# hasnainfarid/Mujoco_Gymnasium_Environments

Hardware: AMD Instinct MI355X
Metric: env steps/sec (whole node), humanoid_soccer 4096 envs/GPU at 1/2/4/8 MI355X (higher is better)
Workload: dtype f64

## Files before the change

### mujoco_gymnasium_environments_amd/csrc/mgx_api.hip

```cpp
#include <hip/hip_runtime.h>

#include <cmath>
#include <cstdio>
#include <cstring>
#include <map>
#include <mutex>
#include <string>
#include <vector>

#include "mgx_internal.h"

using namespace mgx;

MGX_PROF_SETTER(mgx_prof_set_buffer)

namespace {
thread_local std::string g_err;
int fail(int code, const std::string& msg) {
  g_err = msg;
  return code;
}
#define HIPCHK(x) MGX_HIPCHK(x)
}

// ... 543 lines not shown
  p.bcap = 32 + (p.maxE / 4) * (8 + 32 * ((nv + 7) / 8));
  p.tw = MGX_TW;
  p.nobs = nobs;
  size_t off = 0;
  auto take = [&](size_t bytes) { size_t r = off; off = (off + bytes + 255) / 256 * 256; return r; };
  size_t S = (size_t)p.S, NB = (size_t)n_env * (banks > 0 ? banks : 1);
  p.o_ctr = take(64);
  p.o_carry = take(S * p.carry_stride * rb);
  p.o_carryi = take(S * p.carryi_stride * 4);
  p.o_ne = take(S * 4); p.o_blen = take(S * 4); p.o_niter = take(S * 4); p.o_k2list = take(S * 4); p.o_k2big = take(S * 4); p.o_fix = take((size_t)n_env * 4);
  p.hmain = !rk && !cap_env && !p.sqg && !H.pgs_lds_b && p.capE < p.maxE &&
            staged_pgs_lds_bytes(m, p.maxE, pgs_lanes(), 1, mgx_twl(false)) <=
                (H.pgs_wpc == 4 ? staged_pgs_lds_bytes(m, p.capE, pgs_lanes(), 0, mgx_twl(false))
                                : 160 * 1024 / H.pgs_wpc);
  if (p.hmain) p.warena = 0;
  p.split_blocks = 0;
  const int split = H.pgs_split_blocks >= 0 ? H.pgs_split_blocks : split_default;
  if (!rk && !p.sqg && !H.pgs_lds_b && pgs_lanes() == 16 && split > 0) {
    const int one = staged_pgs_lds_bytes(m, p.maxE, 64, 0, mgx_twl(false));
    int main_lds = staged_pgs_lds_bytes(m, p.capE, 16, 0, mgx_twl(false));
    if (p.hmain) main_lds = std::max(main_lds, staged_pgs_lds_bytes(m, p.maxE, 16, 1, mgx_twl(false)));
    const bool b32 = (uint64_t)p.bcap * (uint64_t)rb < (1ull << 32);
    if (b32 && one <= (cap_env ? 160 * 1024 : main_lds)) {
      p.split_blocks = std::min(split, p.capE / 4 + 1);
      p.hmain = 0;
      p.warena = 0;
    }
  }
  p.prio_rows = H.pgs_prio_rows > 0 ? H.pgs_prio_rows : p.capE;
  p.nbk = (p.hmain || p.split_blocks ? p.maxE : p.capE) / 4 + 1;
  p.o_hist = take((size_t)(p.maxE / 4 + 1) * 4);
  p.o_blist = take((size_t)(p.maxE / 4 + 1) * S * 4);
  p.o_scal = take(S * p.maxE * MGX_SCAL * rb);
  p.o_blk = take(S * (p.maxE / 4) * p.tw * 4);
  p.o_B = take(S * (size_t)p.bcap * rb);
  p.o_vout = take(S * 64 * rb);
  p.o_bq = take(NB * nq * rb); p.o_bv = take(NB * nv * rb); p.o_ba = take(NB * nv * rb); p.o_btime = take(NB * rb);
  p.o_bobs = take(NB * nobs * 4); p.o_bprev = take(NB * 6 * rb); p.o_bwind = take(NB * 3 * rb);
  p.o_bk = take(NB * 4); p.o_bep = take(NB * 4); p.o_bwarn = take(NB * 4); p.o_bseed = take(NB * 8);
  int nb = m->precision == MGX_F32 ? m->mf.nbody : m->md.nbody;
  p.maxC = m->Ls.max_ncon;
  p.o_cpos = take(S * 3 * (size_t)p.maxC * rb);
  p.o_tq = take(nq * rb); p.o_tv = take(nv * rb); p.o_ta = take(64 * rb); p.o_tt = take(rb);
  p.o_tx = take(3 * nb * rb); p.o_txq = take(4 * nb * rb); p.o_tsc = take(3 * nb * rb); p.o_tn = take(4);
  p.o_tcg = take(2 * p.maxC * 4); p.o_tcd = take(p.maxC * rb); p.o_tcm = take(p.maxC * rb);
  p.o_rkw = take(S * 4);
  p.o_tscr = take(m->L.gB ? (size_t)m->L.gB_stride * rb : 64);
  if (rk) {
    const int nq4 = (nq + 3) & ~3;
    p.rk_stride = 2 * nq4 + 8 * 64 + 4;
    p.o_rk = take(S * p.rk_stride * rb);
    p.o_rks = take(S * 4);
  }
  if (P) *P = p;
  return off;
}
static size_t make_pipe(const mgx_model* m, void* ws, int n_env, int banks, Pipe* P) {
  return make_staged_pipe(m, ws, n_env, banks, P, false, 80, MGX_PGS_SPLIT_BLOCKS);
}

int mgx::staged_pgs_lds_bytes(const mgx_model* m, int rows, int lps, int sqg, int twl) {
  int rb = m->precision == MGX_F32 ? 4 : 8;
  int nb3 = (rows / 4 + MGX_PGS_RING - 1) / MGX_PGS_RING * MGX_PGS_RING;
  const int spw = 64 / lps;
  const int sq = sqg ? 4 : 4 * MGX_SCAL;
  return spw * (sq * nb3 + 4) * rb + spw * nb3 * 4 * twl + 64;
}
static int pgs_lds_bytes(const mgx_model* m, int rows, int sqg = 0) {
  return staged_pgs_lds_bytes(m, rows, pgs_lanes(), sqg, mgx_twl(false));
}

mgx::Hooks mgx::read_hooks() {
  Hooks h;
  auto get = [](const char* name, int dflt) {
    const char* v = getenv(name);
    return v && *v ? atoi(v) : dflt;
  };
  h.pgs_lds_rows = get("MGX_PGS_LDS_ROWS", 0);
  h.rk_lds_rows = get("MGX_RK_LDS_ROWS", 0);
  h.pgs_single = get("MGX_PGS_SINGLE", 0);
  h.pgs_lds_b = get("MGX_PGS_LDS_B", MGX_PGS_LDS_B) != 0;
  h.pgs_arena = get("MGX_PGS_ARENA", 0);
  h.pgs_lds_pad = get("MGX_PGS_LDS_PAD", 0);
  h.pgs_wide_lds = get("MGX_PGS_WIDE_LDS", 1);
  h.pgs_spw = get("MGX_PGS_SPW", 0);
  h.pgs_prio_rows = get("MGX_PGS_PRIO_ROWS", 0);
  h.pgs_split_blocks = get("MGX_PGS_SPLIT_BLOCKS", -1);
  h.tight_bp = get("MGX_TIGHT_BROADPHASE", -1);
  h.pgs_wpc = get("MGX_PGS_WPC", 4);
  if (h.pgs_wpc < 4 || h.pgs_wpc > 16) h.pgs_wpc = 4;
  h.side_stream = get("MGX_SIDE_STREAM", 1) != 0;
  h.gcon = get("MGX_GCON", 1);
  h.rows_lds = get("MGX_ROWS_LDS", 0);
  return h;
}

struct SideStream {
  hipStream_t s;
  hipEvent_t rows, big;
};
static SideStream* side_stream(hipStream_t st) {
  static std::mutex mu;
  static std::map<std::pair<hipStream_t, int>, SideStream*> cache;
  int dev = 0;
  if (hipGetDevice(&dev) != hipSuccess) return nullptr;
  std::lock_guard<std::mutex> lock(mu);
  auto key = std::make_pair(st, dev);
  auto it = cache.find(key);
  if (it != cache.end()) return it->second;
  SideStream* x = new SideStream{};
  if (hipStreamCreateWithFlags(&x->s, hipStreamNonBlocking) != hipSuccess ||
      hipEventCreateWithFlags(&x->rows, hipEventDisableTiming) != hipSuccess ||
      hipEventCreateWithFlags(&x->big, hipEventDisableTiming) != hipSuccess) {
    delete x;
    x = nullptr;
  }
  cache[key] = x;
  return x;
}

static int settle_lds_bytes(const mgx_model* m, const Pipe& P) {
  int b = pgs_lds_bytes(m, P.maxE);
  if (m->Ls.bytes > b) b = m->Ls.bytes;
  if (m->Lf.bytes > b) b = m->Lf.bytes;
  return b;
}

template <typename T>
static int soccer_step_staged(const mgx_model* m, const DevModel<T>& M, const DevModel<T>& Ms, const DevModel<T>& Mf,
                              const SoccerIds<T>& ids, const mgx_state* s, const mgx_soccer_env* e, const float* action,
                              float* obs, double* reward, uint8_t* terminated, uint8_t* truncated, float* final_obs,
                              int autoreset, uint64_t seed, int env_offset, int n_env, const uint8_t* mask,
                              hipStream_t st) {
  Pipe P;
  int banks = autoreset ? e->banks : 0;
  size_t need = make_pipe(m, e->workspace, n_env, e->banks, &P);
  if (e->workspace_bytes < need) return fail(MGX_E_ARG, "workspace smaller than mgx_soccer_workspace_bytes");
  int slots = n_env * (1 + banks);
  const Hooks& H = m->hooks;
  const int rlds = H.rows_lds > m->Ls.bytes && H.rows_lds <= 64 * 1024 ? H.rows_lds : m->Ls.bytes;
  launch_soccer_rows<T>(Ms, ids, *s, *e, action, n_env, mask, P, banks, slots, rlds, st);
  T scale = (T)1 / (M.meaninertia * (T)(M.nv > 1 ? M.nv : 1));
  const int wgrid = 64 / pgs_lanes() * MGX_PGS_WIDE_GRID, wlds = pgs_lds_bytes(m, P.maxE);
  int mlds = H.pgs_lds_b ? P.arena : pgs_lds_bytes(m, P.capE, P.sqg);
  if (P.hmain) mlds = std::max(mlds, pgs_lds_bytes(m, P.maxE, 1));
  if (P.split_blocks) mlds = std::max(mlds, staged_pgs_lds_bytes(m, P.maxE, 64, 0, mgx_twl(false)));
  if (H.pgs_lds_pad > mlds && H.pgs_lds_pad <= 96 * 1024) mlds = H.pgs_lds_pad;
  if (!H.pgs_lds_b && (P.maxE <= P.capE || P.hmain || P.split_blocks)) {
    launch_pgs<T>(P, slots, mlds, st, M.iterations, M.tolerance, scale, 0, H);
  } else if (SideStream* side = (!H.pgs_lds_b && H.side_stream) ? side_stream(st) : nullptr) {
    HIPCHK(hipEventRecord(side->rows, st));
    HIPCHK(hipStreamWaitEvent(side->s, side->rows, 0));
    launch_pgs<T>(P, wgrid, wlds, side->s, M.iterations, M.tolerance, scale, 1, H);
    HIPCHK(hipEventRecord(side->big, side->s));
    launch_pgs<T>(P, slots, mlds, st, M.iterations, M.tolerance, scale, 0, H);
    HIPCHK(hipStreamWaitEvent(st, side->big, 0));
  } else {
    launch_pgs<T>(P, slots, mlds, st, M.iterations, M.tolerance, scale, 0, H);
    launch_pgs<T>(P, wgrid, wlds, st, M.iterations, M.tolerance, scale, 1, H);
  }
  launch_soccer_finish<T>(Mf, ids, *s, *e, action, obs, reward, terminated, truncated, final_obs, autoreset, seed,
                          env_offset, n_env, mask, P, banks, m->Lf.bytes, st);
  int fgrid = n_env < 256 ? n_env : 256;
  launch_soccer_settle<T>(Ms, Mf, ids, *s, *e, (const T*)nullptr, obs, seed, env_offset, n_env, nullptr, P, SETTLE_FIXUP,
                          fgrid, settle_lds_bytes(m, P), st, M.iterations, M.tolerance, scale);
  HIPCHK(hipGetLastError());
  return MGX_OK;
}

template <typename T>
static int soccer_reset_staged(const mgx_model* m, const DevModel<T>& M, const DevModel<T>& Ms, const DevModel<T>& Mf,
                               const SoccerIds<T>& ids, const mgx_state* s, const mgx_soccer_env* e, const T* draws,
                               float* obs, uint64_t seed, int env_offset, int n_env, const uint8_t* mask, hipStream_t st) {
  Pipe P;
  size_t need = make_pipe(m, e->workspace, n_env, e->banks, &P);
  if (e->workspace_bytes < need) return fail(MGX_E_ARG, "workspace smaller than mgx_soccer_workspace_bytes");
  T scale = (T)1 / (M.meaninertia * (T)(M.nv > 1 ? M.nv : 1));
  launch_soccer_settle<T>(Ms, Mf, ids, *s, *e, draws, obs, seed, env_offset, n_env, mask, P, SETTLE_RESET, n_env,
                          settle_lds_bytes(m, P), st, M.iterations, M.tolerance, scale);
  HIPCHK(hipGetLastError());
  return MGX_OK;
}

template <typename T>
static void fill_ids(SoccerIds<T>& o, const mgx_soccer_ids* ids, const DevModel<T>& M, const mgx_model_desc* unused) {
  (void)unused;
  o.torso = ids->torso; o.ball = ids->ball; o.goalkeeper = ids->goalkeeper; o.ball_geom = ids->ball_geom;
  o.right_foot = ids->right_foot; o.left_foot = ids->left_foot; o.field_geom = ids->field_geom;
  o.ball_qposadr = ids->ball_qposadr; o.ball_dofadr = ids->ball_dofadr; o.gk_qposadr = ids->gk_qposadr;
  o.gk_qfrc_index = ids->gk_dofadr; o.max_episode_steps = ids->max_episode_steps;
  for (int i = 0; i < 25; i++) {
    o.obs_qposadr[i] = ids->obs_jnt_qposadr[i];
    o.obs_dofadr[i] = ids->obs_jnt_dofadr[i];
    o.obs_lo[i] = (T)ids->obs_jnt_range[2 * i];
    o.obs_hi[i] = (T)ids->obs_jnt_range[2 * i + 1];
// ... 180 lines not shown
    hipLaunchKernelGGL((k_soccer<float, 0>), dim3(n_env), dim3(64), m->L.bytes, st, m->mf, m->sf, *s, *e, action,
                       (const float*)nullptr, obs, reward, terminated, truncated, final_obs, autoreset, seed,
                       env_offset, n_env, mask, none, 0);
  else
    hipLaunchKernelGGL((k_soccer<double, 0>), dim3(n_env), dim3(64), m->L.bytes, st, m->md, m->sd, *s, *e, action,
                       (const double*)nullptr, obs, reward, terminated, truncated, final_obs, autoreset, seed,
                       env_offset, n_env, mask, none, 0);
  HIPCHK(hipGetLastError());
  return MGX_OK;
}

int mgx_soccer_reset(const mgx_model* m, const mgx_state* s, const mgx_soccer_env* e, const void* draws, float* obs,
                     uint64_t seed, int env_offset, int n_env, const uint8_t* mask, void* stream) {
  if (!m || !e || !obs) return fail(MGX_E_ARG, "null argument");
  if (!m->soccer_ok) return fail(MGX_E_ARG, "mgx_soccer_configure not called");
  if (!draws && !e->episode) return fail(MGX_E_ARG, "device draws need the episode counter buffer");
  int rc = check_state(s);
  if (rc) return rc;
  if (n_env <= 0) return MGX_OK;
  hipStream_t st = (hipStream_t)stream;
  if (e->workspace) {
    if (!m->staged_ok) return fail(MGX_E_UNSUPPORTED, "staged step: model exceeds the staged solver's capacity");
    if (e->banks < 0 || e->banks > 16) return fail(MGX_E_ARG, "banks must be in [0, 16]");
    if (m->precision == MGX_F32)
      return soccer_reset_staged<float>(m, m->mf, m->mfs, m->mff, m->sf, s, e, (const float*)draws, obs, seed,
                                        env_offset, n_env, mask, st);
    return soccer_reset_staged<double>(m, m->md, m->mds, m->mdf, m->sd, s, e, (const double*)draws, obs, seed,
                                       env_offset, n_env, mask, st);
  }
  Pipe none{};
  if (m->precision == MGX_F32)
    hipLaunchKernelGGL((k_soccer<float, 1>), dim3(n_env), dim3(64), m->L.bytes, st, m->mf, m->sf, *s, *e,
                       (const float*)nullptr, (const float*)draws, obs, (double*)nullptr, (uint8_t*)nullptr,
                       (uint8_t*)nullptr, (float*)nullptr, 0, seed, env_offset, n_env, mask, none, 0);
  else
    hipLaunchKernelGGL((k_soccer<double, 1>), dim3(n_env), dim3(64), m->L.bytes, st, m->md, m->sd, *s, *e,
                       (const float*)nullptr, (const double*)draws, obs, (double*)nullptr, (uint8_t*)nullptr,
                       (uint8_t*)nullptr, (float*)nullptr, 0, seed, env_offset, n_env, mask, none, 0);
  HIPCHK(hipGetLastError());
  return MGX_OK;
}

int64_t mgx_soccer_workspace_bytes(const mgx_model* m, int n_env, int banks) {
  if (!m || n_env <= 0 || banks < 0 || banks > 16) return fail(MGX_E_ARG, "bad argument");
  if (!m->staged_ok) return fail(MGX_E_UNSUPPORTED, "staged step: model exceeds the staged solver's capacity");
  return (int64_t)make_pipe(m, nullptr, n_env, banks, nullptr);
}

int mgx_soccer_workspace_layout(const mgx_model* m, int n_env, int banks, int64_t* out, int n_out) {
  if (!m || !out || n_env <= 0 || banks < 0 || banks > 16 || n_out < 10) return fail(MGX_E_ARG, "bad argument");
  if (!m->staged_ok) return fail(MGX_E_UNSUPPORTED, "staged step: model exceeds the staged solver's capacity");
  Pipe P;
  make_pipe(m, nullptr, n_env, banks, &P);
  const int64_t v[11] = {(int64_t)P.o_ctr, (int64_t)P.o_ne, (int64_t)P.o_k2list, (int64_t)P.o_blk, (int64_t)P.o_B,
                         P.bcap, P.maxE, P.capE, P.S, m->precision == MGX_F32 ? 4 : 8, (int64_t)P.o_k2big};
  for (int i = 0; i < (n_out < 11 ? n_out : 11); i++) out[i] = v[i];
  return MGX_OK;
}

int mgx_soccer_workspace_init(const mgx_model* m, void* workspace, uint64_t bytes, int n_env, int banks, void* stream) {
  if (!m || !workspace || n_env <= 0 || banks < 0 || banks > 16) return fail(MGX_E_ARG, "bad argument");
  Pipe P;
  size_t need = make_pipe(m, workspace, n_env, banks, &P);
  if (bytes < need) return fail(MGX_E_ARG, "workspace smaller than mgx_soccer_workspace_bytes");
  hipStream_t st = (hipStream_t)stream;
  HIPCHK(hipMemsetAsync(workspace, 0, need, st));
  size_t nb = (size_t)n_env * (banks > 0 ? banks : 1);
  HIPCHK(hipMemsetAsync(P.base + P.o_bk, 0xFF, nb * 4, st));
  if (m->precision == MGX_F32)
    hipLaunchKernelGGL(k_soccer_template<float>, dim3(1), dim3(64), m->L.bytes, st, m->mf, P);
  else
    hipLaunchKernelGGL(k_soccer_template<double>, dim3(1), dim3(64), m->L.bytes, st, m->md, P);
  HIPCHK(hipGetLastError());
  return MGX_OK;
}

int mgx_soccer_logic_test(const mgx_model* m, const mgx_soccer_logic_io* io, int n_env, void* stream) {
  if (!m || !io) return fail(MGX_E_ARG, "null argument");
  if (!m->soccer_ok) return fail(MGX_E_ARG, "mgx_soccer_configure not called");
  if (io->max_contacts > m->L.max_ncon) return fail(MGX_E_CAPACITY, "max_contacts exceeds the contact capacity");
  if (n_env <= 0) return MGX_OK;
  hipStream_t st = (hipStream_t)stream;
  if (m->precision == MGX_F32)
    hipLaunchKernelGGL(k_soccer_logic<float>, dim3(n_env), dim3(64), m->L.bytes, st, m->mf, m->sf, *io, n_env);
  else
    hipLaunchKernelGGL(k_soccer_logic<double>, dim3(n_env), dim3(64), m->L.bytes, st, m->md, m->sd, *io, n_env);
  HIPCHK(hipGetLastError());
  return MGX_OK;
}

}
```

### mujoco_gymnasium_environments_amd/csrc/mgx_internal.h

```cpp
#pragma once
#include <hip/hip_runtime.h>

#include <string>

#include "../../include/mgx.h"
#include "mgx_bipedal.h"
#include "mgx_construction.h"
#include "mgx_dancing.h"
#include "mgx_martial.h"
#include "mgx_parkour.h"
#include "mgx_staged.h"

namespace mgx {
struct Hooks {
  int pgs_lds_rows = 0;
  int rk_lds_rows = 0;
  int pgs_single = 0;
  int pgs_lds_b = 0;
  int pgs_arena = 0;
  int pgs_lds_pad = 0;
  int pgs_wide_lds = 1;
  int pgs_spw = 0;
  int pgs_wpc = 4;
  int pgs_prio_rows = 0;
  int pgs_split_blocks = -1;
  int tight_bp = -1;
  int side_stream = 1;
  int gcon = 1;
  int rows_lds = 0;
};
Hooks read_hooks();
struct RayState;
struct SensorState;
}

struct mgx_model {
  mgx::Hooks hooks;
  int precision;
  int device;
  void* dbuf = nullptr;
  size_t dbytes = 0;
  mgx::DevModel<float> mf, mfs, mff;
  mgx::DevModel<double> md, mds, mdf;
  mgx::Layout L, Ls, Lf;
  bool soccer_ok = false;
  mgx::SoccerIds<float> sf;
  mgx::SoccerIds<double> sd;
  bool parkour_ok = false;
  mgx::ParkourIds<float> pkf;
  mgx::ParkourIds<double> pkd;
  bool martial_ok = false;
  mgx::MartialIds ma;
  bool bipedal_ok = false;
  mgx::BipedalIds bp;
  bool dancing_ok = false;
  mgx::DancingIds dn;
  bool assembly_ok = false;
  mgx_assembly_ids as;
  bool construction_ok = false;
  mgx::ConstructionIds cn;
  int npair;
  bool wide = false;
  bool staged_ok = false;
  bool staged_rk_ok = false;
  mgx::RayState* ray = nullptr;
  mgx::SensorState* sensor = nullptr;
};

namespace mgx {
struct DbgOff {
  int xpos, xquat, xipos, subtree_com, cinert, cdof, qM, qLD, geom_xpos, geom_xmat, ncon, con_dist, con_pos,
      con_frame, con_geom, nefc, efc_type, efc_id, efc_pos, efc_margin, efc_R, efc_aref, Bmat, cvel, cdof_dot,
      qfrc_smooth, qacc_smooth, efc_force, qacc, qfrc_constraint, niter, total;
};
inline DbgOff dbg_offsets(int nb, int nv, int nM, int ng, int C, int E) {
  DbgOff o;
  int p = 0;
  auto take = [&](int n) { int r = p; p += n; return r; };
  o.xpos = take(3 * nb); o.xquat = take(4 * nb); o.xipos = take(3 * nb); o.subtree_com = take(3 * nb);
  o.cinert = take(10 * nb); o.cdof = take(6 * nv); o.qM = take(nM); o.qLD = take(nM);
  o.geom_xpos = take(3 * ng); o.geom_xmat = take(9 * ng); o.ncon = take(1); o.con_dist = take(C);
  o.con_pos = take(3 * C); o.con_frame = take(9 * C); o.con_geom = take(2 * C); o.nefc = take(1);
  o.efc_type = take(E); o.efc_id = take(E); o.efc_pos = take(E); o.efc_margin = take(E); o.efc_R = take(E);
  o.efc_aref = take(E); o.Bmat = take(E * nv); o.cvel = take(6 * nb); o.cdof_dot = take(6 * nv);
  o.qfrc_smooth = take(nv); o.qacc_smooth = take(nv); o.efc_force = take(E); o.qacc = take(nv);
  o.qfrc_constraint = take(nv); o.niter = take(1); o.total = p;
  return o;
}
int wide_step(const mgx_model* m, const mgx_state* s, const mgx_frames& fr, int n_env, int nsub, const uint8_t* mask,
              hipStream_t st);
int wide_debug(const mgx_model* m, const mgx_state* s, int n_env, void* dbg, const DbgOff& o, hipStream_t st);
int wide_kernels_configure(const mgx_model* m);
int host_fail(int code, const std::string& msg);
int host_check_state(const mgx_state* s);
int step_kernels_configure(const mgx_model* m);
template <typename T>
void launch_pgs(const Pipe& P, int slots, int lds, hipStream_t st, int maxit, T tol, T scale, int big, const Hooks& h);
int pgs_configure_lds(int precision, int bytes, int wide);
template <typename T>
void launch_soccer_rows(const DevModel<T>& Ms, const SoccerIds<T>& ids, const mgx_state& s, const mgx_soccer_env& ev,
                        const float* action, int n_env, const uint8_t* mask, const Pipe& P, int banks, int slots, int lds,
                        hipStream_t st);
template <typename T>
void launch_soccer_finish(const DevModel<T>& Mf, const SoccerIds<T>& ids, const mgx_state& s, const mgx_soccer_env& ev,
                          const float* action, float* obs, double* reward, uint8_t* terminated, uint8_t* truncated,
                          float* final_obs, int autoreset, uint64_t seed, int env_offset, int n_env, const uint8_t* mask,
                          const Pipe& P, int banks, int lds, hipStream_t st);
template <typename T>
void launch_soccer_settle(const DevModel<T>& Ms, const DevModel<T>& Mf, const SoccerIds<T>& ids, const mgx_state& s,
                          const mgx_soccer_env& ev, const T* draws, float* obs, uint64_t seed, int env_offset, int n_env,
                          const uint8_t* mask, const Pipe& P, int mode, int grid, int lds, hipStream_t st, int maxit, T tol,
                          T scale);
int staged_kernels_configure(int precision, int ls, int lf, int settle);
size_t make_staged_pipe(const mgx_model* m, void* ws, int n_env, int banks, Pipe* P, bool rk, int nobs,
                        int split_default = 0);
int staged_pgs_lds_bytes(const mgx_model* m, int rows, int lps, int sqg, int twl);
int bipedal_staged_configure(const mgx_model* m);
int bipedal_step_staged(const mgx_model* m, const mgx_state* s, const mgx_bipedal_env* e, const float* action, float* obs,
                        double* reward, uint8_t* terminated, uint8_t* truncated, float* final_obs, int autoreset,
                        uint64_t seed, int env_offset, int n_env, const uint8_t* mask, hipStream_t st);
int bipedal_reset_staged(const mgx_model* m, const mgx_state* s, const mgx_bipedal_env* e, const void* draws,
                         float* obs, uint64_t seed, int env_offset, int n_env, const uint8_t* mask, hipStream_t st);
int64_t bipedal_workspace_bytes(const mgx_model* m, int n_env, int banks);
int bipedal_workspace_init(const mgx_model* m, void* workspace, uint64_t bytes, int n_env, int banks, hipStream_t st);
bool parkour_staged_ok(const mgx_model* m);
int parkour_staged_configure(const mgx_model* m);
int parkour_step_staged(const mgx_model* m, const mgx_state* s, const mgx_parkour_env* e, const float* action, float* obs,
                        double* reward, uint8_t* terminated, uint8_t* truncated, float* final_obs, int autoreset,
                        uint64_t seed, int env_offset, int n_env, const uint8_t* mask, hipStream_t st);
int parkour_reset_staged(const mgx_model* m, const mgx_state* s, const mgx_parkour_env* e, const void* draws,
                         float* obs, uint64_t seed, int env_offset, int n_env, const uint8_t* mask, hipStream_t st);
int64_t parkour_workspace_bytes(const mgx_model* m, int n_env, int banks);
int parkour_workspace_init(const mgx_model* m, void* workspace, uint64_t bytes, int n_env, int banks, hipStream_t st);
int pgs_lanes();
void ray_release(mgx_model* m);
void sensor_release(mgx_model* m);
int forward_kernels_configure(const mgx_model* m);
int dyn_kernels_configure(const mgx_model* m);
}

#define MGX_WIDE_MSG "nv > 64: this model runs on the wide (two dofs per lane) kernels only"

#define MGX_HIPCHK(x)                                                                                   \
  do {                                                                                                  \
    hipError_t _e = (x);                                                                                \
    if (_e != hipSuccess) return mgx::host_fail(MGX_E_HIP, std::string(#x) + ": " + hipGetErrorString(_e)); \
  } while (0)

template <typename KernelT>
int mgx_set_lds(KernelT k, int bytes) {
  if (bytes > 64 * 1024) MGX_HIPCHK(hipFuncSetAttribute((const void*)k, hipFuncAttributeMaxDynamicSharedMemorySize, bytes));
  return MGX_OK;
}
```

### mujoco_gymnasium_environments_amd/csrc/mgx_pgs.hip

```cpp
#include "mgx_internal.h"

namespace mgx {

int pgs_lanes() {
  static const int lanes = [] {
    const char* v = getenv("MGX_PGS_LPS");
    const int x = v ? atoi(v) : MGX_PGS_LPS;
    return x == 64 ? 64 : 16;
  }();
  return lanes;
}
template <typename T, int LPS, bool BLDS, bool SQG = false>
static void launch_lps(const Pipe& P, int slots, int lds, hipStream_t st, int maxit, T tol, T scale, int big,
                       int spw_hook, int spw_force = 0) {
  const int spw = spw_force ? spw_force : spw_hook ? spw_hook : 64 / LPS;
  int grid = (slots + (spw < 0 ? -spw : spw) - 1) / (spw < 0 ? -spw : spw);
  switch ((P.dpl + LPS / 8 - 1) / (LPS / 8)) {
#define MGX_PGS_CASE(E)                                                                                          \
    case E:                                                                                                     \
      hipLaunchKernelGGL((k_pgs_groups<T, E, LPS, BLDS, SQG>), dim3(grid), dim3(64), lds, st, P, maxit, tol, scale, spw, \
                         big);                                                                                  \
      break;
    MGX_PGS_CASE(1)
    default:
      if constexpr (LPS == 16) {
        switch ((P.dpl + 1) / 2) { MGX_PGS_CASE(2) MGX_PGS_CASE(3) MGX_PGS_CASE(4) default: break; }
      }
      break;
#undef MGX_PGS_CASE
  }
}

template <typename T>
void launch_pgs(const Pipe& P, int slots, int lds, hipStream_t st, int maxit, T tol, T scale, int big, const Hooks& h) {
  if (big && P.warena > 0 && pgs_lanes() == 16) {
    launch_lps<T, 16, true>(P, MGX_PGS_WIDE_LDS_GRID, P.warena + 64, st, maxit, tol, scale, big, h.pgs_spw, 1);
    return;
  }
  const bool blds = !big && h.pgs_lds_b;
  const int sp = h.pgs_spw;
  if (pgs_lanes() == 64) {
    if (blds) launch_lps<T, 64, true>(P, slots, lds, st, maxit, tol, scale, big, sp);
    else launch_lps<T, 64, false>(P, slots, lds, st, maxit, tol, scale, big, sp);
  } else {
    if (blds) launch_lps<T, 16, true>(P, slots, lds, st, maxit, tol, scale, big, sp);
    else if (P.sqg && !big) launch_lps<T, 16, false, true>(P, slots, lds, st, maxit, tol, scale, big, sp);
    else launch_lps<T, 16, false>(P, slots, lds, st, maxit, tol, scale, big, sp);
  }
}
template void launch_pgs<float>(const Pipe&, int, int, hipStream_t, int, float, float, int, const Hooks&);
template void launch_pgs<double>(const Pipe&, int, int, hipStream_t, int, double, double, int, const Hooks&);

template <typename T>
__global__ void __launch_bounds__(64) k_soccer_rows(DevModel<T> m, SoccerIds<T> ids, mgx_state s, mgx_soccer_env ev,
                                                    const float* action, int n_env, const uint8_t* mask, Pipe P,
                                                    int banks) {
  extern __shared__ __attribute__((aligned(16))) char smem[];
  int b = blockIdx.x;
  int slot;
  Env<T> e;
  if (b < n_env) {
    if (mask && !mask[b]) return;
    env_bind(m, e, smem);
    bind_carry_tail(m, e, P, b);
    load_state(m, e, (T*)s.qpos, (T*)s.qvel, (T*)s.qacc_warmstart, (T*)s.ctrl, (T*)s.qfrc_applied, (T*)s.xfrc_applied,
               (T*)s.time, b);
    soccer_pre(m, e, ids, SoccerAct(action, ev.action_f64, b, m.nu), (T*)ev.prev_ball_pos + 3 * (size_t)b,
               (T*)ev.wind + 3 * (size_t)b);
    slot = b;
  } else {
    int bi = b - n_env;
    if (!banks || bi >= n_env * P.R) return;
    int k = P.at<int>(P.o_bk)[bi];
    if (k < 0 || k >= 10) return;
    env_bind(m, e, smem);
    bind_carry_tail(m, e, P, b);
    bank_load_state(m, e, P, bi);
    slot = b;
  }
  int warn = 0;
  if (any_bad(e.qpos, m.nq)) { reset_env(m, e); warn++; }
  if (any_bad(e.qvel, m.nv)) { reset_env(m, e); warn++; }
  stage_rows(m, e, P, slot, warn);
}

template <typename T>
__global__ void __launch_bounds__(64) k_soccer_bank_finish(DevModel<T> m, SoccerIds<T> ids, int n_env, Pipe P) {
  extern __shared__ __attribute__((aligned(16))) char smem[];
  const int bi = blockIdx.x;
  if (bi >= n_env * P.R) return;
  int k = P.at<int>(P.o_bk)[bi];
  if (k < 0 || k >= 10) return;
  Env<T> e;
  env_bind(m, e, smem);
  const int slot = n_env + bi;
  int warn = load_carry(m, e, P, slot);
  if (!finish_physics(m, e, P, slot)) {
    load_template(m, e, P);
    warn++;
  }
  bank_store_state(m, e, P, bi, warn);
  k++;
  if (k == 10) bank_finalize(m, e, ids, P, bi);
  if (lane_id() == 0) P.at<int>(P.o_bk)[bi] = k;
}

template <typename T>
__global__ void __launch_bounds__(64) k_soccer_finish(DevModel<T> m, SoccerIds<T> ids, mgx_state s, mgx_soccer_env ev,
                                                      const float* action, float* obs, double* reward,
                                                      uint8_t* terminated, uint8_t* truncated, float* final_obs,
                                                      int autoreset, uint64_t seed, int env_offset, int n_env,
                                                      const uint8_t* mask, Pipe P, int banks) {
  extern __shared__ __attribute__((aligned(16))) char smem[];
  int env = blockIdx.x;
  if (env >= n_env) return;
  int l = lane_id();
  if (env == 0 && l == 0) {
    P.ctr()[3] = P.ctr()[1];
    P.ctr()[4] = P.ctr()[2];
    P.ctr()[1] = 0;
    P.ctr()[2] = 0;
  }
  if (env == 0)
    for (int b = lane_id(); b < P.nbk; b += 64) P.at<int>(P.o_hist)[b] = 0;
  Env<T> e;
  env_bind(m, e, smem);
  if (mask && !mask[env]) return;
  int warn = load_carry(m, e, P, env);
  if (!finish_physics(m, e, P, env)) {
    load_template(m, e, P);
    warn++;
  }
  store_state(m, e, (T*)s.qpos, (T*)s.qvel, (T*)s.qacc_warmstart, (T*)s.ctrl, (T*)s.qfrc_applied, (T*)s.xfrc_applied,
              (T*)s.time, env);
  if (l == 0 && s.warning) s.warning[env] += warn;
  if (l == 0 && s.overflow && e.overflow) s.overflow[env] += 1;
  const SoccerAct a(action, ev.action_f64, env, m.nu);
  float* o = obs + (size_t)env * 80;
  bool done = soccer_post(m, e, ids, a, ev.step + env, ev.goal_scored + env, (T*)ev.prev_ball_pos + 3 * (size_t)env,
                          (T*)ev.prev_robot_pos + 3 * (size_t)env, (T*)ev.stats + 5 * (size_t)env, o, reward + env,
                          terminated + env, truncated + env, ev.flags ? ev.flags + 2 * (size_t)env : nullptr);
  if (ev.rollout && l == 0) {
    double* ro = (double*)ev.rollout + 8 * (size_t)env;
    const double ne = e.nefc, it = e.nefc > 0 ? P.at<int>(P.o_niter)[env] : 0;
    ro[0] += reward[env];
    ro[1] += terminated[env];
    ro[2] += truncated[env];
    ro[3] += 1.0;
    ro[4] += ne;
    ro[5] += it;
    ro[6] += ne * ne;
    ro[7] += it * ne * ne;
  }
  if (done && autoreset) {
    if (final_obs)
      for (int i = l; i < 80; i += 64) final_obs[(size_t)env * 80 + i] = o[i];
    __threadfence();
    wsync();
    bool ok = banks && bank_install(m, e, ids, P, s, ev, obs, seed, env_offset, env);
    if (!ok && l == 0) {
      int i = atomicAdd(P.ctr(), 1);
      P.at<int>(P.o_fix)[i] = env * 4 + FIX_RESET;
    }
  }
}


template <typename T>
void launch_soccer_rows(const DevModel<T>& Ms, const SoccerIds<T>& ids, const mgx_state& s, const mgx_soccer_env& ev,
                        const float* action, int n_env, const uint8_t* mask, const Pipe& P, int banks, int slots, int lds,
                        hipStream_t st) {
  hipLaunchKernelGGL(k_soccer_rows<T>, dim3(slots), dim3(64), lds, st, Ms, ids, s, ev, action, n_env, mask, P, banks);
}
template <typename T>
void launch_soccer_finish(const DevModel<T>& Mf, const SoccerIds<T>& ids, const mgx_state& s, const mgx_soccer_env& ev,
                          const float* action, float* obs, double* reward, uint8_t* terminated, uint8_t* truncated,
                          float* final_obs, int autoreset, uint64_t seed, int env_offset, int n_env, const uint8_t* mask,
                          const Pipe& P, int banks, int lds, hipStream_t st) {
  if (banks && P.R > 0)
    hipLaunchKernelGGL(k_soccer_bank_finish<T>, dim3(n_env * P.R), dim3(64), lds, st, Mf, ids, n_env, P);
  hipLaunchKernelGGL(k_soccer_finish<T>, dim3(n_env), dim3(64), lds, st, Mf, ids, s, ev, action, obs, reward, terminated,
                     truncated, final_obs, autoreset, seed, env_offset, n_env, mask, P, banks);
}
template <typename T>
void launch_soccer_settle(const DevModel<T>& Ms, const DevModel<T>& Mf, const SoccerIds<T>& ids, const mgx_state& s,
                          const mgx_soccer_env& ev, const T* draws, float* obs, uint64_t seed, int env_offset, int n_env,
                          const uint8_t* mask, const Pipe& P, int mode, int grid, int lds, hipStream_t st, int maxit, T tol,
                          T scale) {
#define MGX_SETTLE(E, L)                                                                                            \
  hipLaunchKernelGGL((k_soccer_settle<T, E, L>), dim3(grid), dim3(64), lds, st, Ms, Mf, ids, s, ev, draws, obs, seed, \
                     env_offset, n_env, mask, P, mode, maxit, tol, scale)
  if (pgs_lanes() == 64) {
    MGX_SETTLE(1, 64);
  } else {
    switch ((P.dpl + 1) / 2) {
      case 1: MGX_SETTLE(1, 16); break;
      case 2: MGX_SETTLE(2, 16); break;
      case 3: MGX_SETTLE(3, 16); break;
      default: MGX_SETTLE(4, 16); break;
    }
  }
#undef MGX_SETTLE
}
#define MGX_STAGED_INST(T)                                                                                              \
  template void launch_soccer_rows<T>(const DevModel<T>&, const SoccerIds<T>&, const mgx_state&, const mgx_soccer_env&, \
                                      const float*, int, const uint8_t*, const Pipe&, int, int, int, hipStream_t);      \
  template void launch_soccer_finish<T>(const DevModel<T>&, const SoccerIds<T>&, const mgx_state&,                      \
                                        const mgx_soccer_env&, const float*, float*, double*, uint8_t*, uint8_t*, float*, \
                                        int, uint64_t, int, int, const uint8_t*, const Pipe&, int, int, hipStream_t);     \
  template void launch_soccer_settle<T>(const DevModel<T>&, const DevModel<T>&, const SoccerIds<T>&, const mgx_state&, \
                                        const mgx_soccer_env&, const T*, float*, uint64_t, int, int, const uint8_t*,    \
                                        const Pipe&, int, int, int, hipStream_t, int, T, T);
MGX_STAGED_INST(float)
MGX_STAGED_INST(double)
#undef MGX_STAGED_INST

int staged_kernels_configure(int precision, int ls, int lf, int settle) {
  int rc = 0;
#define MGX_SETTLE_SET(T) \
  rc |= mgx_set_lds(k_soccer_settle<T, 1, 16>, settle) | mgx_set_lds(k_soccer_settle<T, 2, 16>, settle) | \
        mgx_set_lds(k_soccer_settle<T, 3, 16>, settle) | mgx_set_lds(k_soccer_settle<T, 4, 16>, settle) | \
        mgx_set_lds(k_soccer_settle<T, 1, 64>, settle);
  if (precision == MGX_F32) {
    rc |= mgx_set_lds(k_soccer_rows<float>, ls > 64 * 1024 ? ls : 64 * 1024) | mgx_set_lds(k_soccer_finish<float>, lf) |
          mgx_set_lds(k_soccer_bank_finish<float>, lf);
    MGX_SETTLE_SET(float)
  } else {
    rc |= mgx_set_lds(k_soccer_rows<double>, ls > 64 * 1024 ? ls : 64 * 1024) | mgx_set_lds(k_soccer_finish<double>, lf) |
          mgx_set_lds(k_soccer_bank_finish<double>, lf);
    MGX_SETTLE_SET(double)
  }
#undef MGX_SETTLE_SET
  return rc;
}

int pgs_configure_lds(int precision, int pl, int wl) {
  int rc = 0;
#define MGX_PGS_SET(T, E, L)                                                                            \
  rc |= mgx_set_lds(k_pgs_groups<T, E, L, true>, pl > wl ? pl : wl) | mgx_set_lds(k_pgs_groups<T, E, L, false>, pl) | \
        mgx_set_lds(k_pgs_groups<T, E, L, false, true>, pl);
#define MGX_PGS_SET_ALL(T) \
  MGX_PGS_SET(T, 1, 16) MGX_PGS_SET(T, 2, 16) MGX_PGS_SET(T, 3, 16) MGX_PGS_SET(T, 4, 16) MGX_PGS_SET(T, 1, 64)
  if (precision == MGX_F32) { MGX_PGS_SET_ALL(float) } else { MGX_PGS_SET_ALL(double) }
#undef MGX_PGS_SET_ALL
#undef MGX_PGS_SET
  return rc;
}

}

MGX_PROF_SETTER(mgx_prof_set_buffer_pgs)
```

### mujoco_gymnasium_environments_amd/csrc/mgx_staged.h

```cpp
#pragma once
#include "mgx_soccer.h"

namespace mgx {

#define MGX_SCAL 5
#define MGX_SQ(k, i) (4 * (k) + (i))
#define MGX_TW 4
__host__ __device__ constexpr int mgx_twl(bool dofb) { return dofb ? 4 : 8; }
#define MGX_PGS_LPS 16
#define MGX_PGS_LDS_B 0
#define MGX_PGS_RING 2
#define MGX_PGS_RING_LDS 2
#define MGX_PGS_LDS_ROWS 192
#define MGX_PGS_SPLIT_BLOCKS 40
#define MGX_PGS_WIDE_GRID 256
#define MGX_PGS_WIDE_LDS_GRID 32
#define MGX_PGS_ARENA_F64 49152
#define MGX_PGS_ARENA_F32 32768
enum { FIX_RESET = 2 };

struct Pipe {
  char* base;
  int N, R, S, maxE, dpl, nv;
  int carry_stride;
  int carryi_stride;
  int bcap;
  int capE;
  int arena;
  int sqg;
  int prio_rows;
  int hmain;
  int split_blocks;
  int warena;
  size_t o_cpos;
  size_t o_carry, o_carryi, o_ne, o_blen, o_niter, o_k2list, o_k2big, o_ctr, o_fix, o_scal, o_blk, o_B, o_vout;
  int nbk;
  size_t o_hist, o_blist;
  size_t o_bq, o_bv, o_ba, o_btime, o_bobs, o_bprev, o_bwind, o_bk, o_bep, o_bwarn, o_bseed;
  size_t o_tq, o_tv, o_ta, o_tt, o_tx, o_txq, o_tsc, o_tn, o_tcg, o_tcd, o_tcm;
  int maxC;
  int tw;
  int nobs;
  int rk_stride;
  size_t o_rk, o_rks, o_rkw, o_tscr;
  template <typename X> __device__ __forceinline__ X* at(size_t off) const { return reinterpret_cast<X*>(base + off); }
  __device__ __forceinline__ int* ctr() const { return at<int>(o_ctr); }
};

template <typename T>
__device__ __forceinline__ void bind_carry_tail(const DevModel<T>& m, Env<T>& e, const Pipe& P, int slot) {
  if (m.L.carry_lds < m.L.carry_reals) {
    T* cr = P.at<T>(P.o_carry) + (size_t)slot * P.carry_stride;
    e.xfrc = cr + (m.L.xfrc - m.L.qpos);
    e.qMH = cr + (m.L.qMH - m.L.qpos);
    e.con_mu = cr + (m.L.con_mu - m.L.qpos);
  }
  if (m.L.gcon) e.con_pos = P.at<T>(P.o_cpos) + (size_t)slot * 3 * P.maxC;
}

template <typename T>
__device__ __forceinline__ int rows_plan(const DevModel<T>& m, Env<T>& e, int* nlim_out, int* ncon_out) {
  int l = lane_id();
  const int maxE = m.L.max_nefc;
  int nlim = 0;
  for (int base = 0; base < m.njnt; base += 64) {
    int j = base + l;
    bool lo = false, hi = false;
    if (j < m.njnt && m.jnt_limited[j] && (m.jnt_type[j] == JHINGE || m.jnt_type[j] == JSLIDE)) {
      T val = e.qpos[m.jnt_qposadr[j]], margin = m.jnt_margin[j];
      lo = val - m.jnt_range[2 * j] < margin;
      hi = m.jnt_range[2 * j + 1] - val < margin;
    }
    int total;
    int off = wave_excl_scan((int)lo + (int)hi, &total);
    int r = nlim + off;
    if (lo) { if (r < maxE) e.efc_id[r] = 2 * j; r++; }
    if (hi) { if (r < maxE) e.efc_id[r] = 2 * j + 1; }
    nlim += total;
  }
  if (nlim > maxE) { nlim = maxE; e.overflow |= 4; }
  int nlim4 = (nlim + 3) & ~3;
  int ncf = e.ncon;
  if (nlim4 + 4 * ncf > maxE) { ncf = (maxE - nlim4) / 4; e.overflow |= 4; }
  *nlim_out = nlim;
  *ncon_out = ncf;
  wsync();
  return nlim4 + 4 * ncf;
}

template <typename T>
__device__ __forceinline__ void rows_impedance(const DevModel<T>& m, Env<T>& e, int ne, int nlim, int nlim4, T* scal) {
  const int l = lane_id();
  for (int r = l; r < ne; r += 64) {
    const T *solref = nullptr, *solimp = nullptr;
    T pos = 0, margin = 0, diag = 0;
    if (r < nlim) {
      int code = e.efc_id[r];
// ... 892 lines not shown
    e.con_geom[2 * k + 1] = P.at<int>(P.o_tcg)[2 * k + 1];
    e.con_dist[k] = P.at<T>(P.o_tcd)[k];
    e.con_mu[k] = P.at<T>(P.o_tcm)[k];
  }
  e.qacc_ws = l < m.nv ? P.at<T>(P.o_ta)[l] : (T)0;
  e.qfrc_applied = 0;
  e.time = P.at<T>(P.o_tt)[0];
  wsync();
}

template <typename T>
__device__ __forceinline__ bool finish_physics(const DevModel<T>& m, Env<T>& e, const Pipe& P, int slot) {
  int l = lane_id();
  const bool dl = l < m.nv;
  if (e.nefc > 0) {
    T v = dl ? P.at<T>(P.o_vout)[(size_t)slot * 64 + l] : (T)0;
    T D = dl ? e.qLD[m.dof_Madr[l]] : (T)1;
    T sqrtD = sqrt(D);
    T z = dl ? v / sqrtD : (T)0;
    z = solve_L(m, e, e.qLD, z);
    e.qacc = e.qacc_smooth + z;
    e.qfrc_constraint = mul_LT(m, e, e.qLD, dl ? sqrtD * v : (T)0);
  } else {
    e.qacc = e.qacc_smooth;
    e.qfrc_constraint = 0;
  }
  if (ballot(dl && isbad(e.qacc)) != 0ull) return false;
  e.qacc_ws = e.qacc;
  euler(m, e);
  return true;
}

template <typename T>
__device__ __forceinline__ void copy_g(T* dst, const T* src, int n) {
  for (int k = lane_id(); k < n; k += 64) dst[k] = src[k];
}

template <typename T>
__device__ __forceinline__ void bank_init_draws(const DevModel<T>& m, Env<T>& e, const SoccerIds<T>& ids, const Pipe& P,
                                                int bi, int episode, uint64_t seed) {
  int l = lane_id();
  soccer_apply_reset(m, e, ids, e.vec1, P.at<T>(P.o_bwind) + 3 * (size_t)bi);
  copy_g(P.at<T>(P.o_bq) + (size_t)bi * m.nq, e.qpos, m.nq);
  if (l < m.nv) {
    P.at<T>(P.o_bv)[(size_t)bi * m.nv + l] = 0;
    P.at<T>(P.o_ba)[(size_t)bi * m.nv + l] = 0;
  }
  if (l == 0) {
    P.at<T>(P.o_btime)[bi] = 0;
    P.at<int>(P.o_bwarn)[bi] = 0;
    P.at<int>(P.o_bep)[bi] = episode;
    P.at<uint64_t>(P.o_bseed)[bi] = seed;
    P.at<int>(P.o_bk)[bi] = 0;
  }
  wsync();
}
template <typename T>
__device__ __forceinline__ void bank_init(const DevModel<T>& m, Env<T>& e, const SoccerIds<T>& ids, const Pipe& P, int env,
                                          int b, int episode, uint64_t seed, int env_offset) {
  soccer_philox_draws(seed, (uint32_t)(env_offset + env), (uint32_t)episode, ids.n_noise, e.vec1);
  wsync();
  bank_init_draws(m, e, ids, P, env * P.R + b, episode, seed);
}

template <typename T>
__device__ __forceinline__ void bank_finalize(const DevModel<T>& m, Env<T>& e, const SoccerIds<T>& ids, const Pipe& P, int bi) {
  soccer_obs(m, e, ids, 0, P.at<float>(P.o_bobs) + (size_t)bi * 80);
  int l = lane_id();
  T* pv = P.at<T>(P.o_bprev) + (size_t)bi * 6;
  if (l < 3) { pv[l] = e.xpos[3 * ids.ball + l]; pv[3 + l] = e.xpos[3 * ids.torso + l]; }
}

template <typename T>
__device__ __forceinline__ void bank_store_state(const DevModel<T>& m, Env<T>& e, const Pipe& P, int bi, int warn) {
  wsync();
  int l = lane_id();
  copy_g(P.at<T>(P.o_bq) + (size_t)bi * m.nq, e.qpos, m.nq);
  if (l < m.nv) {
    P.at<T>(P.o_bv)[(size_t)bi * m.nv + l] = e.qvel[l];
    P.at<T>(P.o_ba)[(size_t)bi * m.nv + l] = e.qacc_ws;
  }
  if (l == 0) {
    P.at<T>(P.o_btime)[bi] = e.time;
    P.at<int>(P.o_bwarn)[bi] += warn;
  }
}

template <typename T>
__device__ __forceinline__ void bank_load_state(const DevModel<T>& m, Env<T>& e, const Pipe& P, int bi) {
  int l = lane_id();
  const T* q = P.at<T>(P.o_bq) + (size_t)bi * m.nq;
  for (int k = l; k < m.nq; k += 64) e.qpos[k] = q[k];
  for (int k = l; k < m.nv; k += 64) e.qvel[k] = P.at<T>(P.o_bv)[(size_t)bi * m.nv + k];
  for (int k = l; k < m.nu; k += 64) e.ctrl[k] = 0;
  for (int k = l; k < 6 * m.nbody; k += 64) e.xfrc[k] = 0;
  e.qacc_ws = l < m.nv ? P.at<T>(P.o_ba)[(size_t)bi * m.nv + l] : (T)0;
  e.qfrc_applied = 0;
  e.time = P.at<T>(P.o_btime)[bi];
  wsync();
}

template <typename T>
__device__ __forceinline__ void bank_copy_live(const DevModel<T>& m, const Pipe& P, mgx_state s, mgx_soccer_env ev,
                                               float* obs, int env, int bi, int E) {
  int l = lane_id();
  copy_g((T*)s.qpos + (size_t)env * m.nq, P.at<T>(P.o_bq) + (size_t)bi * m.nq, m.nq);
// ... 128 lines not shown
```

Measured before the change: 1.715 million.

## Run autoreset bank pipeline on a separate low-priority stream

Splits the staged soccer step so that live-env rows and PGS run on the main stream while the reset-bank rows, PGS and bank-finish run concurrently on a low-priority side stream, using separate counters and lists in the workspace. A per-bank staging flag records which banks ran so bank-finish does not need to recheck the step counter. This is meant to hide the bank work behind the live-env solve instead of serialising it into one large grid. It adds extra workspace, events and cross-stream synchronisation, and the change in launch shapes and priorities could reduce occupancy or cause contention.

After: 1.770 million, median of 6. 3.2% higher.

```diff
diff --git a/mujoco_gymnasium_environments_amd/csrc/mgx_api.hip b/mujoco_gymnasium_environments_amd/csrc/mgx_api.hip
--- a/mujoco_gymnasium_environments_amd/csrc/mgx_api.hip
+++ b/mujoco_gymnasium_environments_amd/csrc/mgx_api.hip
@@ -619,6 +619,11 @@
     p.o_rk = take(S * p.rk_stride * rb);
     p.o_rks = take(S * 4);
   }
+  p.o_ctr2 = take(64);
+  p.o_hist2 = take((size_t)(p.maxE / 4 + 1) * 4);
+  p.o_blist2 = take((size_t)(p.maxE / 4 + 1) * NB * 4);
+  p.o_k2list2 = take(NB * 4); p.o_k2big2 = take(NB * 4);
+  p.o_bstg = take(NB * 4);
   if (P) *P = p;
   return off;
 }
@@ -657,6 +662,8 @@
   h.pgs_wpc = get("MGX_PGS_WPC", 4);
   if (h.pgs_wpc < 4 || h.pgs_wpc > 16) h.pgs_wpc = 4;
   h.side_stream = get("MGX_SIDE_STREAM", 1) != 0;
+  h.bank_stream = get("MGX_BANK_STREAM", -1);
+  if (h.bank_stream < -1 || h.bank_stream > 2) h.bank_stream = 0;
   h.gcon = get("MGX_GCON", 1);
   h.rows_lds = get("MGX_ROWS_LDS", 0);
   return h;
@@ -686,6 +693,42 @@
   return x;
 }
 
+struct BankStream {
+  hipStream_t s;
+  hipEvent_t entry, rows, live, done;
+};
+static BankStream* bank_stream(hipStream_t st) {
+  static std::mutex mu;
+  static std::map<std::pair<hipStream_t, int>, BankStream*> cache;
+  int dev = 0;
+  if (hipGetDevice(&dev) != hipSuccess) return nullptr;
+  std::lock_guard<std::mutex> lock(mu);
+  auto key = std::make_pair(st, dev);
+  auto it = cache.find(key);
+  if (it != cache.end()) return it->second;
+  BankStream* x = new BankStream{};
+  int least = 0, greatest = 0;
+  if (hipDeviceGetStreamPriorityRange(&least, &greatest) != hipSuccess ||
+      hipStreamCreateWithPriority(&x->s, hipStreamNonBlocking, least) != hipSuccess ||
+      hipEventCreateWithFlags(&x->entry, hipEventDisableTiming) != hipSuccess ||
+      hipEventCreateWithFlags(&x->rows, hipEventDisableTiming) != hipSuccess ||
+      hipEventCreateWithFlags(&x->live, hipEventDisableTiming) != hipSuccess ||
+      hipEventCreateWithFlags(&x->done, hipEventDisableTiming) != hipSuccess) {
+    (void)hipGetLastError();
+    delete x;
+    x = nullptr;
+  }
+  cache[key] = x;
+  return x;
+}
+static Pipe bank_view(const Pipe& P) {
+  Pipe B = P;
+  B.o_ctr = P.o_ctr2; B.o_hist = P.o_hist2; B.o_blist = P.o_blist2; B.o_k2list = P.o_k2list2; B.o_k2big = P.o_k2big2;
+  B.S = P.N * (P.R > 0 ? P.R : 1);
+  B.prio_rows = P.maxE;
+  return B;
+}
+
 static int settle_lds_bytes(const mgx_model* m, const Pipe& P) {
   int b = pgs_lds_bytes(m, P.maxE);
   if (m->Ls.bytes > b) b = m->Ls.bytes;
@@ -706,8 +749,47 @@
   int slots = n_env * (1 + banks);
   const Hooks& H = m->hooks;
   const int rlds = H.rows_lds > m->Ls.bytes && H.rows_lds <= 64 * 1024 ? H.rows_lds : m->Ls.bytes;
+  T scale = (T)1 / (M.meaninertia * (T)(M.nv > 1 ? M.nv : 1));
+  int bmode = banks > 0 && H.side_stream && !H.pgs_lds_b && !H.pgs_single &&
+                      (P.maxE <= P.capE || P.hmain || P.split_blocks)
+                  ? (H.bank_stream >= 0 ? H.bank_stream : m->precision == MGX_F32 ? 0 : MGX_BANK_STREAM) : 0;
+  BankStream* bs = bmode ? bank_stream(st) : nullptr;
+  if (bs) {
+    const Pipe B = bank_view(P);
+    const int nbank = n_env * P.R;
+    if (!H.pgs_prio_rows && P.split_blocks) P.prio_rows = 4 * P.split_blocks - 1;
+    int mlds = pgs_lds_bytes(m, P.capE, P.sqg);
+    if (P.hmain) mlds = std::max(mlds, pgs_lds_bytes(m, P.maxE, 1));
+    if (P.split_blocks) mlds = std::max(mlds, staged_pgs_lds_bytes(m, P.maxE, 64, 0, mgx_twl(false)));
+    if (H.pgs_lds_pad > mlds && H.pgs_lds_pad <= 96 * 1024) mlds = H.pgs_lds_pad;
+    HIPCHK(hipEventRecord(bs->entry, st));
+    launch_soccer_rows<T>(Ms, ids, *s, *e, action, n_env, mask, P, 0, n_env, rlds, st);
+    HIPCHK(hipStreamWaitEvent(bs->s, bs->entry, 0));
+    launch_soccer_rows<T>(Ms, ids, *s, *e, action, n_env, nullptr, B, banks, nbank, rlds, bs->s, n_env);
+    if (bmode == 2) HIPCHK(hipEventRecord(bs->rows, bs->s));
+    launch_pgs<T>(B, nbank, mlds, bs->s, M.iterations, M.tolerance, scale, 0, H);
+    if (bmode == 1) {
+      launch_soccer_bank_finish<T>(Mf, ids, n_env, B, 1, m->Lf.bytes, bs->s);
+      HIPCHK(hipEventRecord(bs->done, bs->s));
+    }
+    launch_pgs<T>(P, n_env, mlds, st, M.iterations, M.tolerance, scale, 0, H);
+    HIPCHK(hipStreamWaitEvent(st, bmode == 1 ? bs->done : bs->rows, 0));
+    launch_soccer_finish<T>(Mf, ids, *s, *e, action, obs, reward, terminated, truncated, final_obs, autoreset, seed,
+                            env_offset, n_env, mask, P, banks, m->Lf.bytes, st, false);
+    int fgrid = n_env < 256 ? n_env : 256;
+    launch_soccer_settle<T>(Ms, Mf, ids, *s, *e, (const T*)nullptr, obs, seed, env_offset, n_env, nullptr, P,
+                            SETTLE_FIXUP, fgrid, settle_lds_bytes(m, P), st, M.iterations, M.tolerance, scale);
+    if (bmode == 2) {
+      HIPCHK(hipEventRecord(bs->live, st));
+      HIPCHK(hipStreamWaitEvent(bs->s, bs->live, 0));
+      launch_soccer_bank_finish<T>(Mf, ids, n_env, B, 1, m->Lf.bytes, bs->s);
+      HIPCHK(hipEventRecord(bs->done, bs->s));
+      HIPCHK(hipStreamWaitEvent(st, bs->done, 0));
+    }
+    HIPCHK(hipGetLastError());
+    return MGX_OK;
+  }
   launch_soccer_rows<T>(Ms, ids, *s, *e, action, n_env, mask, P, banks, slots, rlds, st);
-  T scale = (T)1 / (M.meaninertia * (T)(M.nv > 1 ? M.nv : 1));
   const int wgrid = 64 / pgs_lanes() * MGX_PGS_WIDE_GRID, wlds = pgs_lds_bytes(m, P.maxE);
   int mlds = H.pgs_lds_b ? P.arena : pgs_lds_bytes(m, P.capE, P.sqg);
   if (P.hmain) mlds = std::max(mlds, pgs_lds_bytes(m, P.maxE, 1));
@@ -994,9 +1076,10 @@
   if (!m->staged_ok) return fail(MGX_E_UNSUPPORTED, "staged step: model exceeds the staged solver's capacity");
   Pipe P;
   make_pipe(m, nullptr, n_env, banks, &P);
-  const int64_t v[11] = {(int64_t)P.o_ctr, (int64_t)P.o_ne, (int64_t)P.o_k2list, (int64_t)P.o_blk, (int64_t)P.o_B,
-                         P.bcap, P.maxE, P.capE, P.S, m->precision == MGX_F32 ? 4 : 8, (int64_t)P.o_k2big};
-  for (int i = 0; i < (n_out < 11 ? n_out : 11); i++) out[i] = v[i];
+  const int64_t v[13] = {(int64_t)P.o_ctr, (int64_t)P.o_ne, (int64_t)P.o_k2list, (int64_t)P.o_blk, (int64_t)P.o_B,
+                         P.bcap, P.maxE, P.capE, P.S, m->precision == MGX_F32 ? 4 : 8, (int64_t)P.o_k2big,
+                         (int64_t)P.o_ctr2, (int64_t)P.o_k2list2};
+  for (int i = 0; i < (n_out < 13 ? n_out : 13); i++) out[i] = v[i];
   return MGX_OK;
 }
 
diff --git a/mujoco_gymnasium_environments_amd/csrc/mgx_internal.h b/mujoco_gymnasium_environments_amd/csrc/mgx_internal.h
--- a/mujoco_gymnasium_environments_amd/csrc/mgx_internal.h
+++ b/mujoco_gymnasium_environments_amd/csrc/mgx_internal.h
@@ -26,6 +26,7 @@
   int pgs_split_blocks = -1;
   int tight_bp = -1;
   int side_stream = 1;
+  int bank_stream = 0;
   int gcon = 1;
   int rows_lds = 0;
 };
@@ -100,12 +101,15 @@
 template <typename T>
 void launch_soccer_rows(const DevModel<T>& Ms, const SoccerIds<T>& ids, const mgx_state& s, const mgx_soccer_env& ev,
                         const float* action, int n_env, const uint8_t* mask, const Pipe& P, int banks, int slots, int lds,
-                        hipStream_t st);
+                        hipStream_t st, int slot0 = 0);
+template <typename T>
+void launch_soccer_bank_finish(const DevModel<T>& Mf, const SoccerIds<T>& ids, int n_env, const Pipe& P, int lists,
+                               int lds, hipStream_t st);
 template <typename T>
 void launch_soccer_finish(const DevModel<T>& Mf, const SoccerIds<T>& ids, const mgx_state& s, const mgx_soccer_env& ev,
                           const float* action, float* obs, double* reward, uint8_t* terminated, uint8_t* truncated,
                           float* final_obs, int autoreset, uint64_t seed, int env_offset, int n_env, const uint8_t* mask,
-                          const Pipe& P, int banks, int lds, hipStream_t st);
+                          const Pipe& P, int banks, int lds, hipStream_t st, bool bank_too = true);
 template <typename T>
 void launch_soccer_settle(const DevModel<T>& Ms, const DevModel<T>& Mf, const SoccerIds<T>& ids, const mgx_state& s,
                           const mgx_soccer_env& ev, const T* draws, float* obs, uint64_t seed, int env_offset, int n_env,
diff --git a/mujoco_gymnasium_environments_amd/csrc/mgx_pgs.hip b/mujoco_gymnasium_environments_amd/csrc/mgx_pgs.hip
--- a/mujoco_gymnasium_environments_amd/csrc/mgx_pgs.hip
+++ b/mujoco_gymnasium_environments_amd/csrc/mgx_pgs.hip
@@ -54,9 +54,9 @@
 template <typename T>
 __global__ void __launch_bounds__(64) k_soccer_rows(DevModel<T> m, SoccerIds<T> ids, mgx_state s, mgx_soccer_env ev,
                                                     const float* action, int n_env, const uint8_t* mask, Pipe P,
-                                                    int banks) {
+                                                    int banks, int b0) {
   extern __shared__ __attribute__((aligned(16))) char smem[];
-  int b = blockIdx.x;
+  int b = b0 + blockIdx.x;
   int slot;
   Env<T> e;
   if (b < n_env) {
@@ -72,7 +72,9 @@
     int bi = b - n_env;
     if (!banks || bi >= n_env * P.R) return;
     int k = P.at<int>(P.o_bk)[bi];
-    if (k < 0 || k >= 10) return;
+    const bool run = k >= 0 && k < 10;
+    if (lane_id() == 0) P.at<int>(P.o_bstg)[bi] = run;
+    if (!run) return;
     env_bind(m, e, smem);
     bind_carry_tail(m, e, P, b);
     bank_load_state(m, e, P, bi);
@@ -85,12 +87,22 @@
 }
 
 template <typename T>
-__global__ void __launch_bounds__(64) k_soccer_bank_finish(DevModel<T> m, SoccerIds<T> ids, int n_env, Pipe P) {
+__global__ void __launch_bounds__(64) k_soccer_bank_finish(DevModel<T> m, SoccerIds<T> ids, int n_env, Pipe P,
+                                                           int lists) {
   extern __shared__ __attribute__((aligned(16))) char smem[];
   const int bi = blockIdx.x;
+  if (lists && bi == 0) {
+    if (lane_id() == 0) {
+      P.ctr()[3] = P.ctr()[1];
+      P.ctr()[4] = P.ctr()[2];
+      P.ctr()[1] = 0;
+      P.ctr()[2] = 0;
+    }
+    for (int b = lane_id(); b < P.nbk; b += 64) P.at<int>(P.o_hist)[b] = 0;
+  }
   if (bi >= n_env * P.R) return;
+  if (!P.at<int>(P.o_bstg)[bi]) return;
   int k = P.at<int>(P.o_bk)[bi];
-  if (k < 0 || k >= 10) return;
   Env<T> e;
   env_bind(m, e, smem);
   const int slot = n_env + bi;
@@ -102,7 +114,10 @@
   bank_store_state(m, e, P, bi, warn);
   k++;
   if (k == 10) bank_finalize(m, e, ids, P, bi);
-  if (lane_id() == 0) P.at<int>(P.o_bk)[bi] = k;
+  if (lane_id() == 0) {
+    P.at<int>(P.o_bk)[bi] = k;
+    P.at<int>(P.o_bstg)[bi] = 0;
+  }
 }
 
 template <typename T>
@@ -169,16 +184,21 @@
 template <typename T>
 void launch_soccer_rows(const DevModel<T>& Ms, const SoccerIds<T>& ids, const mgx_state& s, const mgx_soccer_env& ev,
                         const float* action, int n_env, const uint8_t* mask, const Pipe& P, int banks, int slots, int lds,
-                        hipStream_t st) {
-  hipLaunchKernelGGL(k_soccer_rows<T>, dim3(slots), dim3(64), lds, st, Ms, ids, s, ev, action, n_env, mask, P, banks);
+                        hipStream_t st, int slot0) {
+  hipLaunchKernelGGL(k_soccer_rows<T>, dim3(slots), dim3(64), lds, st, Ms, ids, s, ev, action, n_env, mask, P, banks,
+                     slot0);
+}
+template <typename T>
+void launch_soccer_bank_finish(const DevModel<T>& Mf, const SoccerIds<T>& ids, int n_env, const Pipe& P, int lists,
+                               int lds, hipStream_t st) {
+  hipLaunchKernelGGL(k_soccer_bank_finish<T>, dim3(n_env * P.R), dim3(64), lds, st, Mf, ids, n_env, P, lists);
 }
 template <typename T>
 void launch_soccer_finish(const DevModel<T>& Mf, const SoccerIds<T>& ids, const mgx_state& s, const mgx_soccer_env& ev,
                           const float* action, float* obs, double* reward, uint8_t* terminated, uint8_t* truncated,
                           float* final_obs, int autoreset, uint64_t seed, int env_offset, int n_env, const uint8_t* mask,
-                          const Pipe& P, int banks, int lds, hipStream_t st) {
-  if (banks && P.R > 0)
-    hipLaunchKernelGGL(k_soccer_bank_finish<T>, dim3(n_env * P.R), dim3(64), lds, st, Mf, ids, n_env, P);
+                          const Pipe& P, int banks, int lds, hipStream_t st, bool bank_too) {
+  if (bank_too && banks && P.R > 0) launch_soccer_bank_finish<T>(Mf, ids, n_env, P, 0, lds, st);
   hipLaunchKernelGGL(k_soccer_finish<T>, dim3(n_env), dim3(64), lds, st, Mf, ids, s, ev, action, obs, reward, terminated,
                      truncated, final_obs, autoreset, seed, env_offset, n_env, mask, P, banks);
 }
@@ -204,10 +224,13 @@
 }
 #define MGX_STAGED_INST(T)                                                                                              \
   template void launch_soccer_rows<T>(const DevModel<T>&, const SoccerIds<T>&, const mgx_state&, const mgx_soccer_env&, \
-                                      const float*, int, const uint8_t*, const Pipe&, int, int, int, hipStream_t);      \
+                                      const float*, int, const uint8_t*, const Pipe&, int, int, int, hipStream_t, int); \
+  template void launch_soccer_bank_finish<T>(const DevModel<T>&, const SoccerIds<T>&, int, const Pipe&, int, int,       \
+                                             hipStream_t);                                                              \
   template void launch_soccer_finish<T>(const DevModel<T>&, const SoccerIds<T>&, const mgx_state&,                      \
                                         const mgx_soccer_env&, const float*, float*, double*, uint8_t*, uint8_t*, float*, \
-                                        int, uint64_t, int, int, const uint8_t*, const Pipe&, int, int, hipStream_t);     \
+                                        int, uint64_t, int, int, const uint8_t*, const Pipe&, int, int, hipStream_t,      \
+                                        bool);                                                                            \
   template void launch_soccer_settle<T>(const DevModel<T>&, const DevModel<T>&, const SoccerIds<T>&, const mgx_state&, \
                                         const mgx_soccer_env&, const T*, float*, uint64_t, int, int, const uint8_t*,    \
                                         const Pipe&, int, int, int, hipStream_t, int, T, T);
diff --git a/mujoco_gymnasium_environments_amd/csrc/mgx_staged.h b/mujoco_gymnasium_environments_amd/csrc/mgx_staged.h
--- a/mujoco_gymnasium_environments_amd/csrc/mgx_staged.h
+++ b/mujoco_gymnasium_environments_amd/csrc/mgx_staged.h
@@ -13,6 +13,7 @@
 #define MGX_PGS_RING_LDS 2
 #define MGX_PGS_LDS_ROWS 192
 #define MGX_PGS_SPLIT_BLOCKS 40
+#define MGX_BANK_STREAM 1
 #define MGX_PGS_WIDE_GRID 256
 #define MGX_PGS_WIDE_LDS_GRID 32
 #define MGX_PGS_ARENA_F64 49152
@@ -43,6 +44,7 @@
   int nobs;
   int rk_stride;
   size_t o_rk, o_rks, o_rkw, o_tscr;
+  size_t o_ctr2, o_hist2, o_blist2, o_k2list2, o_k2big2, o_bstg;
   template <typename X> __device__ __forceinline__ X* at(size_t off) const { return reinterpret_cast<X*>(base + off); }
   __device__ __forceinline__ int* ctr() const { return at<int>(o_ctr); }
 };
@@ -1041,6 +1043,7 @@
     P.at<int>(P.o_bep)[bi] = episode;
     P.at<uint64_t>(P.o_bseed)[bi] = seed;
     P.at<int>(P.o_bk)[bi] = 0;
+    P.at<int>(P.o_bstg)[bi] = 0;
   }
   wsync();
 }
```
